# sonbui25/Multimodal-Aspect-Category-Sentiment-Analysis

Measured on AMD Instinct MI355X. Metric: train samples/sec (fwd+bwd+step) FCMF seq128x36ROI, higher is better.
Workload: dtype bf16; 1 GPU; FCMF-base fine-tune step, BASELINE configs[1]: batch 64 reviews x 6 aspects per GPU, seq 128, 7 images x (49 patches + 36 ROIs), precomputed ResNet-152 features, dropout 0.1, clip 1.0 + 4-group AdamW + linear schedule; global_batch=64, per_gpu_batch=64, seq_len=128, parallelism=dp1, sample_unit=1 review = 6 aspect forwards

## Files before the change

### multimodal-aspect-category-sentiment-analysis_amd/csrc/attn_mfma.hip

```cpp
#include "attn_tiles.h"
#include <cstdlib>


template <int NKT>
__device__ __forceinline__ void attn_mfma_fwd_tile(const AttnMfmaParams& P, int g, int h, int q0, int lane, const bf16x8 (&qf)[2][2],
                                                   const char* Ks, const char* Vs, const float* mask_lds = nullptr) {
  constexpr int NKF = 8 * NKT;
  const float* mrow = P.mask ? P.mask + (int64_t)g * P.Tk : nullptr;
  int nvalid = P.Tk;
  if (mask_lds || mrow) {
    int last = -1;
#pragma unroll
    for (int i = 0; i < 2 * NKT; ++i) {
      const int key = 64 * i + lane;
      const bool live = key < P.Tk && (mask_lds ? mask_lds[key] : mrow[key]) > -1e30f;
      const unsigned long long b = __ballot(live);
      if (b) last = 64 * i + 63 - __builtin_clzll(b);
    }
    nvalid = last >= 0 ? last + 1 : P.Tk;
  }
  f32x4 sc[NKF][2];
#pragma unroll
  for (int kf = 0; kf < NKF; ++kf)
#pragma unroll
    for (int f = 0; f < 2; ++f) sc[kf][f] = f32x4{0.f, 0.f, 0.f, 0.f};
#pragma unroll
  for (int s = 0; s < 2; ++s)
#pragma unroll
    for (int kf = 0; kf < NKF; ++kf) {
      if (16 * kf >= nvalid) continue;
      const bf16x8 ka = frag_row64(Ks, 16 * kf, s, lane);
#pragma unroll
      for (int f = 0; f < 2; ++f) sc[kf][f] = __builtin_amdgcn_mfma_f32_16x16x32_bf16(ka, qf[f][s], sc[kf][f], 0, 0, 0);
    }
  const float inv_keep = P.p > 0.f ? 1.0f / (1.0f - P.p) : 1.0f;
#pragma unroll
  for (int f = 0; f < 2; ++f) {
    const int q = q0 + 16 * f + (lane & 15);
    float m = -INFINITY;
#pragma unroll
    for (int kf = 0; kf < NKF; ++kf) {
      if (16 * kf >= nvalid) continue;
#pragma unroll
      for (int r = 0; r < 4; ++r) {
        const int key = 16 * kf + 4 * (lane >> 4) + r;
        float s = -INFINITY;
        if (key < P.Tk) s = sc[kf][f][r] * P.scale + (mask_lds ? mask_lds[key] : (mrow ? mrow[key] : 0.f));
        sc[kf][f][r] = s;
        m = fmaxf(m, s);
      }
    }
    m = fmaxf(m, __shfl_xor(m, 16, 64));
    m = fmaxf(m, __shfl_xor(m, 32, 64));
    float sum = 0.f;
#pragma unroll
    for (int kf = 0; kf < NKF; ++kf) {
      if (16 * kf >= nvalid) continue;
#pragma unroll
      for (int r = 0; r < 4; ++r) {
        const float e = __expf(sc[kf][f][r] - m);
        sc[kf][f][r] = e;
        sum += e;
      }
    }
    sum += __shfl_xor(sum, 16, 64);
    sum += __shfl_xor(sum, 32, 64);
    const float inv = 1.0f / sum;
    if (q < P.Tq && (lane >> 4) == 0 && P.lse) P.lse[((int64_t)g * P.heads + h) * P.Tq + q] = m + __logf(sum);
#pragma unroll
    for (int kf = 0; kf < NKF; ++kf) {
      if (16 * kf >= nvalid) continue;
      float dm[4] = {1.f, 1.f, 1.f, 1.f};
      if (P.p > 0.f)
        dropout_mult4(P.seed, ((uint64_t)g * P.heads + h) * P.Tq * P.Tk + (__umul24((unsigned)q, (unsigned)P.Tk) + (unsigned)(16 * kf + 4 * (lane >> 4))),
                      P.p, inv_keep, dm);
#pragma unroll
      for (int r = 0; r < 4; ++r) sc[kf][f][r] = sc[kf][f][r] * inv * dm[r];
    }
  }
  f32x4 oc[4][2];
#pragma unroll
  for (int df = 0; df < 4; ++df)
#pragma unroll
    for (int f = 0; f < 2; ++f) oc[df][f] = f32x4{0.f, 0.f, 0.f, 0.f};
#pragma unroll
  for (int s = 0; s < 4 * NKT; ++s) {
    if (32 * s >= nvalid) continue;
    bf16x8 pb[2];
#pragma unroll
    for (int f = 0; f < 2; ++f)
#pragma unroll
      for (int r = 0; r < 4; ++r) { pb[f][r] = (bf16_t)sc[2 * s][f][r]; pb[f][4 + r] = (bf16_t)sc[2 * s + 1][f][r]; }
#pragma unroll
    for (int df = 0; df < 4; ++df) {
      const bf16x8 va = frag_tr64p(Vs, 16 * df, s, lane);
#pragma unroll
      for (int f = 0; f < 2; ++f) oc[df][f] = __builtin_amdgcn_mfma_f32_16x16x32_bf16(va, pb[f], oc[df][f], 0, 0, 0);
    }
  }
#pragma unroll
  for (int f = 0; f < 2; ++f) {
    const int q = q0 + 16 * f + (lane & 15);
    if (q < P.Tq) {
      bf16_t* orow = P.out + ((int64_t)g * P.Tq + q) * P.ldo + h * AD + 4 * (lane >> 4);
#pragma unroll
      for (int df = 0; df < 4; ++df) store4(orow + 16 * df, oc[df][f]);
    }
  }
}

template <int NKT>
__device__ __forceinline__ void attn_mfma_fwd_body(const AttnMfmaParams& P) {
  extern __shared__ __attribute__((aligned(16))) char smem[];
  char* Ks = smem;
  char* Vs = smem + NKT * TILE_B;
  const int tid = threadIdx.x, lane = tid & 63, w = tid >> 6;
  const int g = blockIdx.x / P.heads, h = blockIdx.x % P.heads;
  const int q0 = blockIdx.y * AT + w * 32;
  const bf16_t* kbase_p = P.k + (int64_t)g * P.Tk * P.ldk + h * AD;
  const bf16_t* vbase_p = P.v + (int64_t)g * P.Tk * P.ldk + h * AD;
  const TileRegs kt = load_tile(kbase_p, P.ldk, P.Tk, tid);
  const TileRegs vt = load_tile(vbase_p, P.ldk, P.Tk, tid);
  bf16x8 qf[2][2];
  load_q_frags(P, g, h, q0, lane, qf);
  store_tile<false>(Ks, kt, tid);
  store_tile<true>(Vs, vt, tid);
  if constexpr (NKT == 2) {
    const TileRegs kt2 = load_tile(kbase_p + (int64_t)AT * P.ldk, P.ldk, P.Tk - AT, tid);
    const TileRegs vt2 = load_tile(vbase_p + (int64_t)AT * P.ldk, P.ldk, P.Tk - AT, tid);
    store_tile<false>(Ks + TILE_B, kt2, tid);
    store_tile<true>(Vs + TILE_B, vt2, tid);
  }
  __syncthreads();
  attn_mfma_fwd_tile<NKT>(P, g, h, q0, lane, qf, Ks, Vs);
}

__global__ __launch_bounds__(256, 2) void attn_mfma_fwd_persist_kernel(AttnMfmaParams P, int ntiles, int qtiles) {
  extern __shared__ __attribute__((aligned(16))) char smem[];
  const int tid = threadIdx.x, lane = tid & 63, w = tid >> 6;
  auto where = [&](int tile, int& g, int& h, int& q0) {
    const int gh = tile / qtiles;
    g = gh / P.heads; h = gh - g * P.heads; q0 = (tile - gh * qtiles) * AT + w * 32;
  };
  constexpr int BUF = 2 * TILE_B + 512;
  int tile = blockIdx.x;
  if (tile >= ntiles) return;
  int g, h, q0;
  where(tile, g, h, q0);
  bf16x8 qf[2][2];
  auto mask_of = [&](int gg) { return (P.mask && tid < P.Tk) ? P.mask[(int64_t)gg * P.Tk + tid] : 0.f; };
  {
    const TileRegs kt = load_tile(P.k + (int64_t)g * P.Tk * P.ldk + h * AD, P.ldk, P.Tk, tid);
    const TileRegs vt = load_tile(P.v + (int64_t)g * P.Tk * P.ldk + h * AD, P.ldk, P.Tk, tid);
    const float mv = mask_of(g);
    load_q_frags(P, g, h, q0, lane, qf);
    store_tile<false>(smem, kt, tid);
    store_tile<true>(smem + TILE_B, vt, tid);
    if (tid < AT) reinterpret_cast<float*>(smem + 2 * TILE_B)[tid] = mv;
  }
  __syncthreads();
  int cur = 0;
  for (;;) {
    const int nxt = tile + gridDim.x;
    const bool more = nxt < ntiles;
    int g2 = g, h2 = h, q2 = q0;
    TileRegs kt, vt;
    bf16x8 qn[2][2];
    float mv = 0.f;
    if (more) {
      where(nxt, g2, h2, q2);
      kt = load_tile(P.k + (int64_t)g2 * P.Tk * P.ldk + h2 * AD, P.ldk, P.Tk, tid);
      vt = load_tile(P.v + (int64_t)g2 * P.Tk * P.ldk + h2 * AD, P.ldk, P.Tk, tid);
      mv = mask_of(g2);
      load_q_frags(P, g2, h2, q2, lane, qn);
    }
    const char* buf = smem + cur * BUF;
    attn_mfma_fwd_tile<1>(P, g, h, q0, lane, qf, buf, buf + TILE_B, reinterpret_cast<const float*>(buf + 2 * TILE_B));
    if (!more) break;
    cur ^= 1;
    store_tile<false>(smem + cur * BUF, kt, tid);
    store_tile<true>(smem + cur * BUF + TILE_B, vt, tid);
    if (tid < AT) reinterpret_cast<float*>(smem + cur * BUF + 2 * TILE_B)[tid] = mv;
#pragma unroll
    for (int f = 0; f < 2; ++f)
#pragma unroll
      for (int s2 = 0; s2 < 2; ++s2) qf[f][s2] = qn[f][s2];
    g = g2; h = h2; q0 = q2; tile = nxt;
    __syncthreads();
  }
}

__global__ __launch_bounds__(256, 3) void attn_mfma_fwd_kernel(AttnMfmaParams P) { attn_mfma_fwd_body<1>(P); }
__global__ __launch_bounds__(256, 2) void attn_mfma_fwd256_kernel(AttnMfmaParams P) { attn_mfma_fwd_body<2>(P); }

template <int NQT, int NKT>
__device__ __forceinline__ void attn_mfma_bwd_body(const AttnMfmaParams& P) {
  extern __shared__ __attribute__((aligned(16))) char smem[];
  char* Qs = smem;
  char* dOs = Qs + NQT * TILE_B;
  char* Ks = dOs + NQT * TILE_B;
  char* Vs = Ks + NKT * TILE_B;
  char* PdT = Vs + NKT * TILE_B;
  char* dST = PdT + TILE_B / 2;
  const int tid = threadIdx.x, lane = tid & 63, w = tid >> 6;
  const int g = blockIdx.x / P.heads, h = blockIdx.x % P.heads;
  const int64_t qbase = (int64_t)g * P.Tq, kbase = (int64_t)g * P.Tk;
  float dl4[NQT][2][4], lse4[NQT][2][4];
  {
    TileRegs tq[NQT], td[NQT];
#pragma unroll
    for (int qt = 0; qt < NQT; ++qt) {
      tq[qt] = load_tile(P.q + (qbase + qt * AT) * P.ldq + h * AD, P.ldq, P.Tq - qt * AT, tid);
      td[qt] = load_tile(P.dout + (qbase + qt * AT) * P.ldo + h * AD, P.ldo, P.Tq - qt * AT, tid);
    }
    TileRegs tk = load_tile(P.k + kbase * P.ldk + h * AD, P.ldk, P.Tk, tid);
    TileRegs tv = load_tile(P.v + kbase * P.ldk + h * AD, P.ldk, P.Tk, tid);
#pragma unroll
    for (int qt = 0; qt < NQT; ++qt) {
      const int q = qt * AT + 32 * w + (lane >> 1), half = lane & 1;
      float sd = 0.f;
      if (q < P.Tq) {
        const bf16_t* a = P.dout + (qbase + q) * P.ldo + h * AD + 32 * half;
        const bf16_t* b = P.o + (qbase + q) * P.ldo + h * AD + 32 * half;
#pragma unroll
        for (int i = 0; i < 4; ++i) {
          const bf16x8 x = *reinterpret_cast<const bf16x8*>(a + 8 * i);
          const bf16x8 y = *reinterpret_cast<const bf16x8*>(b + 8 * i);
#pragma unroll
          for (int j = 0; j < 8; ++j) sd += (float)x[j] * (float)y[j];
        }
      }
      sd += __shfl_xor(sd, 1, 64);
#pragma unroll
      for (int f = 0; f < 2; ++f)
#pragma unroll
        for (int r = 0; r < 4; ++r) {
          const int ql = 16 * f + 4 * (lane >> 4) + r;
          dl4[qt][f][r] = __shfl(sd, 2 * ql, 64);
          const int q2 = qt * AT + 32 * w + ql;
          lse4[qt][f][r] = q2 < P.Tq ? P.lse[((int64_t)g * P.heads + h) * P.Tq + q2] : 0.f;
        }
    }
#pragma unroll
    for (int qt = 0; qt < NQT; ++qt) {
      store_tile<false>(Qs + qt * TILE_B, tq[qt], tid);
      store_tile<false>(dOs + qt * TILE_B, td[qt], tid);
    }
    store_tile<false>(Ks, tk, tid);
    store_tile<false>(Vs, tv, tid);
    if constexpr (NKT == 2) {
      tk = load_tile(P.k + (kbase + AT) * P.ldk + h * AD, P.ldk, P.Tk - AT, tid);
      tv = load_tile(P.v + (kbase + AT) * P.ldk + h * AD, P.ldk, P.Tk - AT, tid);
      store_tile<false>(Ks + TILE_B, tk, tid);
      store_tile<false>(Vs + TILE_B, tv, tid);
    }
  }
  __syncthreads();

  const float inv_keep = P.p > 0.f ? 1.0f / (1.0f - P.p) : 1.0f;
  const uint64_t drop_base = ((uint64_t)g * P.heads + h) * P.Tq * P.Tk;
  const float* mrow = P.mask ? P.mask + kbase : nullptr;
  float score_scale = P.scale;
  bf16x8 qa[NQT][2][2], da[NQT][2][2], oT[NQT][4], qT[NQT][4];
  f32x4 aQ[NQT][4][2];
#pragma unroll
  for (int qt = 0; qt < NQT; ++qt) {
#pragma unroll
    for (int f = 0; f < 2; ++f)
#pragma unroll
      for (int s = 0; s < 2; ++s) {
        qa[qt][f][s] = frag_row64(Qs + qt * TILE_B, 32 * w + 16 * f, s, lane);
        da[qt][f][s] = frag_row64(dOs + qt * TILE_B, 32 * w + 16 * f, s, lane);
// ... 114 lines not shown
      for (int s = 0; s < 4; ++s)
#pragma unroll
        for (int kf = 0; kf < 2; ++kf) {
          const bf16x8 pb = frag_row128(PdT, 16 * kf, s, lane);
          const bf16x8 sb = frag_row128(dST, 16 * kf, s, lane);
          aV[kf] = __builtin_amdgcn_mfma_f32_16x16x32_bf16(oT[qt][s], pb, aV[kf], 0, 0, 0);
          aK[kf] = __builtin_amdgcn_mfma_f32_16x16x32_bf16(qT[qt][s], sb, aK[kf], 0, 0, 0);
        }
      __syncthreads();
    }
    const int dcol = h * AD + 16 * w + 4 * (lane >> 4);
    cV += aV[0] + aV[1];
    cK += aK[0] + aK[1];
#pragma unroll
    for (int kf = 0; kf < 2; ++kf) {
      const int key = 32 * c + 16 * kf + (lane & 15);
      if (key < P.Tk) {
        store4(P.dv + (kbase + key) * P.ldk + dcol, aV[kf]);
        f32x4 t = aK[kf];
        t[0] *= P.scale; t[1] *= P.scale; t[2] *= P.scale; t[3] *= P.scale;
        store4(P.dk + (kbase + key) * P.ldk + dcol, t);
      }
    }
  }
  for (int c = nchunks; c < nchunks_all; ++c) {
    const int dcol = h * AD + 16 * w + 4 * (lane >> 4);
#pragma unroll
    for (int kf = 0; kf < 2; ++kf) {
      const int key = 32 * c + 16 * kf + (lane & 15);
      if (key < P.Tk) {
        store4(P.dv + (kbase + key) * P.ldk + dcol, f32x4{0.f, 0.f, 0.f, 0.f});
        store4(P.dk + (kbase + key) * P.ldk + dcol, f32x4{0.f, 0.f, 0.f, 0.f});
      }
    }
  }
#pragma unroll
  for (int qt = 0; qt < NQT; ++qt)
#pragma unroll
    for (int f = 0; f < 2; ++f) {
      const int x = qt * AT + 32 * w + 16 * f + (lane & 15);
      if (x < P.Tq) {
        const int dcol = h * AD + 4 * (lane >> 4);
#pragma unroll
        for (int df = 0; df < 4; ++df) {
          f32x4 t = aQ[qt][df][f];
          t[0] *= P.scale; t[1] *= P.scale; t[2] *= P.scale; t[3] *= P.scale;
          store4(P.dq + (qbase + x) * P.ldq + dcol + 16 * df, t);
        }
      }
    }
  if (P.colsum) {
    const int HD = P.heads * AD;
    float* row = P.colsum + (int64_t)g * 3 * HD + h * AD;
#pragma unroll
    for (int r = 0; r < 4; ++r) { cV[r] = row16_sum(cV[r]); cK[r] = row16_sum(cK[r]); }
    if ((lane & 15) == 0) {
      const int d0 = 16 * w + 4 * (lane >> 4);
#pragma unroll
      for (int r = 0; r < 4; ++r) { row[2 * HD + d0 + r] = cV[r]; row[HD + d0 + r] = cK[r] * P.scale; }
    }
    float* red = reinterpret_cast<float*>(PdT);
#pragma unroll
    for (int df = 0; df < 4; ++df) {
      f32x4 t = f32x4{0.f, 0.f, 0.f, 0.f};
#pragma unroll
      for (int qt = 0; qt < NQT; ++qt)
#pragma unroll
        for (int f = 0; f < 2; ++f) t += aQ[qt][df][f];
#pragma unroll
      for (int r = 0; r < 4; ++r) t[r] = row16_sum(t[r]);
      if ((lane & 15) == 0) {
#pragma unroll
        for (int r = 0; r < 4; ++r) red[w * 64 + 16 * df + 4 * (lane >> 4) + r] = t[r];
      }
    }
    __syncthreads();
    if (tid < 64) row[tid] = (red[tid] + red[64 + tid] + red[128 + tid] + red[192 + tid]) * P.scale;
  }
}

__global__ __launch_bounds__(256, 2) void attn_mfma_bwd_kernel(AttnMfmaParams P) { attn_mfma_bwd_body<1, 1>(P); }
__global__ __launch_bounds__(256, 1) void attn_mfma_bwd256_kernel(AttnMfmaParams P) { attn_mfma_bwd_body<2, 2>(P); }

static bool al16(const void* p) { return (reinterpret_cast<uintptr_t>(p) & 15) == 0; }

extern "C" int fcmf_attn_mfma_fwd(const void* q, const void* k, const void* v, const float* mask, void* out, float* lse,
                                  int G, int heads, int Tq, int Tk, int64_t ldq, int64_t ldk, int64_t ldo, float scale,
                                  float dropout_p, uint64_t seed, void* stream) {
  if (!q || !k || !v || !out || G <= 0 || heads <= 0 || Tq <= 0 || Tk <= 0) return FCMF_ERR_ARG;
  if (Tk > 2 * AT || ldq % 8 || ldk % 8 || ldo % 4 || !al16(q) || !al16(k) || !al16(v) || !al16(out)) return FCMF_ERR_UNSUPPORTED;
  AttnMfmaParams P{};
  P.q = (const bf16_t*)q; P.k = (const bf16_t*)k; P.v = (const bf16_t*)v; P.mask = mask; P.out = (bf16_t*)out; P.lse = lse;
  P.G = G; P.heads = heads; P.Tq = Tq; P.Tk = Tk; P.ldq = ldq; P.ldk = ldk; P.ldo = ldo;
  P.scale = scale; P.p = dropout_p; P.seed = seed;
  const dim3 grid(G * heads, (Tq + AT - 1) / AT);
  if (Tk > AT) {
    const int smem = 4 * TILE_B;
    static bool attr2 = false;
    return fcmf_launch_flagged(&attr2, attn_mfma_fwd256_kernel, grid, dim3(256), smem, reinterpret_cast<hipStream_t>(stream), P);
  }
  const int ntiles = (int)(grid.x * grid.y);
  static const bool no_persist = getenv("FCMF_ATTN_NO_PERSIST") != nullptr;
  if (ntiles >= 4 * 512 && !no_persist) {
    const int smem = 2 * (2 * TILE_B + 512);
    static bool attr3 = false;
    return fcmf_launch_flagged(&attr3, attn_mfma_fwd_persist_kernel, dim3(512), dim3(256), smem, reinterpret_cast<hipStream_t>(stream), P, ntiles, (int)grid.y);
  }
  const int smem = 2 * TILE_B;
  static bool attr = false;
  return fcmf_launch_flagged(&attr, attn_mfma_fwd_kernel, grid, dim3(256), smem, reinterpret_cast<hipStream_t>(stream), P);
}

extern "C" int fcmf_attn_mfma_bwd(const void* q, const void* k, const void* v, const float* mask, const void* out,
                                  const void* dout, const float* lse, void* dq, void* dk, void* dv, int G, int heads,
                                  int Tq, int Tk, int64_t ldq, int64_t ldk, int64_t ldo, float scale, float dropout_p,
                                  uint64_t seed, float* colsum, void* stream) {
  if (!q || !k || !v || !out || !dout || !lse || !dq || !dk || !dv || G <= 0 || heads <= 0 || Tq <= 0 || Tk <= 0) return FCMF_ERR_ARG;
  if (Tk > 2 * AT || Tq > 2 * AT || ldq % 8 || ldk % 8 || ldo % 8 || !al16(q) || !al16(k) || !al16(v) || !al16(out) || !al16(dout) ||
      !al16(dq) || !al16(dk) || !al16(dv))
    return FCMF_ERR_UNSUPPORTED;
  AttnMfmaParams P{};
  P.q = (const bf16_t*)q; P.k = (const bf16_t*)k; P.v = (const bf16_t*)v; P.mask = mask; P.o = (const bf16_t*)out;
  P.dout = (const bf16_t*)dout; P.lse = const_cast<float*>(lse); P.dq = (bf16_t*)dq; P.dk = (bf16_t*)dk; P.dv = (bf16_t*)dv;
  P.G = G; P.heads = heads; P.Tq = Tq; P.Tk = Tk; P.ldq = ldq; P.ldk = ldk; P.ldo = ldo;
  P.scale = scale; P.p = dropout_p; P.seed = seed; P.colsum = colsum;
  if (Tk > AT || Tq > AT) {
    const int smem = 9 * TILE_B;
    static bool attr2 = false;
    return fcmf_launch_flagged(&attr2, attn_mfma_bwd256_kernel, dim3(G * heads), dim3(256), smem, reinterpret_cast<hipStream_t>(stream), P);
  }
  const int smem = 5 * TILE_B;
  static bool attr = false;
  return fcmf_launch_flagged(&attr, attn_mfma_bwd_kernel, dim3(G * heads), dim3(256), smem, reinterpret_cast<hipStream_t>(stream), P);
}
```

### multimodal-aspect-category-sentiment-analysis_amd/csrc/attn_tiles.h

```cpp
#pragma once
#include "common.h"

constexpr int AD = 64;
constexpr int AT = 128;
constexpr int TILE_B = AT * AD * 2;

__device__ __forceinline__ int vkey(int r) { return ((r >> 1) & 1) | (((r >> 3) & 1) << 1); }
__device__ __forceinline__ int off64(int r, int c8) { return r * 128 + ((((c8 >> 1) ^ vkey(r))) << 5) + ((c8 & 1) << 4); }
__device__ __forceinline__ int key16(int r) { return ((r & 7) << 1) ^ (((r >> 3) & 1) * 9); }
__device__ __forceinline__ int off128(int r, int ch) { return r * 256 + ((ch ^ key16(r)) << 4); }
__device__ __forceinline__ int offp(int r, int ch) { return r * 256 + ((ch ^ (r & 15)) << 4); }

__device__ __forceinline__ int off64p(int r, int c8) { return r * 128 + ((((c8 >> 1) ^ ((r >> 1) & 3))) << 5) + ((c8 & 1) << 4); }

typedef bf16x4 __attribute__((address_space(3))) * lds_v4_t;

__device__ __forceinline__ void stage_tile(char* lds, const bf16_t* __restrict__ src, int64_t ld, int rows, int tid) {
#pragma unroll
  for (int i = 0; i < 4; ++i) {
    const int c = tid + 256 * i, r = c >> 3, c8 = c & 7;
    uint4 v = make_uint4(0, 0, 0, 0);
    if (r < rows) v = *reinterpret_cast<const uint4*>(src + (int64_t)r * ld + c8 * 8);
    *reinterpret_cast<uint4*>(lds + off64(r, c8)) = v;
  }
}
__device__ __forceinline__ void stage_tile_p(char* lds, const bf16_t* __restrict__ src, int64_t ld, int rows, int tid) {
#pragma unroll
  for (int i = 0; i < 4; ++i) {
    const int c = tid + 256 * i, r = c >> 3, c8 = c & 7;
    uint4 v = make_uint4(0, 0, 0, 0);
    if (r < rows) v = *reinterpret_cast<const uint4*>(src + (int64_t)r * ld + c8 * 8);
    *reinterpret_cast<uint4*>(lds + off64p(r, c8)) = v;
  }
}
__device__ __forceinline__ bf16x8 frag_tr64p(const char* lds, int c0, int s, int lane) {
  const int g4 = lane >> 4, i16 = lane & 15, q4 = i16 >> 2, p = i16 & 3;
  const int r = 32 * s + 4 * g4 + q4, c8 = (c0 >> 3) + (p >> 1);
  bf16x4 lo = __builtin_amdgcn_ds_read_tr16_b64_v4bf16((lds_v4_t)(lds + off64p(r, c8) + (p & 1) * 8));
  bf16x4 hi = __builtin_amdgcn_ds_read_tr16_b64_v4bf16((lds_v4_t)(lds + off64p(r + 16, c8) + (p & 1) * 8));
  bf16x8 o;
  o[0] = lo[0]; o[1] = lo[1]; o[2] = lo[2]; o[3] = lo[3]; o[4] = hi[0]; o[5] = hi[1]; o[6] = hi[2]; o[7] = hi[3];
  return o;
}
struct TileRegs { uint4 v[4]; };
__device__ __forceinline__ TileRegs load_tile(const bf16_t* __restrict__ src, int64_t ld, int rows, int tid) {
  TileRegs t;
#pragma unroll
  for (int i = 0; i < 4; ++i) {
    const int c = tid + 256 * i, r = c >> 3, c8 = c & 7;
    t.v[i] = make_uint4(0, 0, 0, 0);
    if (r < rows) t.v[i] = *reinterpret_cast<const uint4*>(src + (int64_t)r * ld + c8 * 8);
  }
  return t;
}
template <bool PERMUTED>
__device__ __forceinline__ void store_tile(char* lds, const TileRegs& t, int tid) {
#pragma unroll
  for (int i = 0; i < 4; ++i) {
    const int c = tid + 256 * i, r = c >> 3, c8 = c & 7;
    *reinterpret_cast<uint4*>(lds + (PERMUTED ? off64p(r, c8) : off64(r, c8))) = t.v[i];
  }
}
__device__ __forceinline__ bf16x8 frag_row64(const char* lds, int x0, int s, int lane) {
  return *reinterpret_cast<const bf16x8*>(lds + off64(x0 + (lane & 15), 4 * s + (lane >> 4)));
}
__device__ __forceinline__ bf16x8 frag_tr64(const char* lds, int c0, int s, int lane) {
  const int g4 = lane >> 4, i16 = lane & 15, q4 = i16 >> 2, p = i16 & 3;
  const int r = 32 * s + 8 * g4 + q4, c8 = (c0 >> 3) + (p >> 1);
  bf16x4 lo = __builtin_amdgcn_ds_read_tr16_b64_v4bf16((lds_v4_t)(lds + off64(r, c8) + (p & 1) * 8));
  bf16x4 hi = __builtin_amdgcn_ds_read_tr16_b64_v4bf16((lds_v4_t)(lds + off64(r + 4, c8) + (p & 1) * 8));
  bf16x8 o;
  o[0] = lo[0]; o[1] = lo[1]; o[2] = lo[2]; o[3] = lo[3]; o[4] = hi[0]; o[5] = hi[1]; o[6] = hi[2]; o[7] = hi[3];
  return o;
}
__device__ __forceinline__ bf16x8 frag_row128(const char* lds, int x0, int s, int lane) {
  return *reinterpret_cast<const bf16x8*>(lds + off128(x0 + (lane & 15), 4 * s + (lane >> 4)));
}
__device__ __forceinline__ bf16x8 frag_tr128(const char* lds, int c0, int s, int lane) {
  const int g4 = lane >> 4, i16 = lane & 15, q4 = i16 >> 2, p = i16 & 3;
  const int r = 32 * s + 8 * g4 + q4, ch = (c0 >> 3) + (p >> 1);
  bf16x4 lo = __builtin_amdgcn_ds_read_tr16_b64_v4bf16((lds_v4_t)(lds + off128(r, ch) + (p & 1) * 8));
  bf16x4 hi = __builtin_amdgcn_ds_read_tr16_b64_v4bf16((lds_v4_t)(lds + off128(r + 4, ch) + (p & 1) * 8));
  bf16x8 o;
  o[0] = lo[0]; o[1] = lo[1]; o[2] = lo[2]; o[3] = lo[3]; o[4] = hi[0]; o[5] = hi[1]; o[6] = hi[2]; o[7] = hi[3];
  return o;
}
__device__ __forceinline__ void store4(bf16_t* p, f32x4 v) {
  bf16x4 o;
  o[0] = (bf16_t)v[0]; o[1] = (bf16_t)v[1]; o[2] = (bf16_t)v[2]; o[3] = (bf16_t)v[3];
  *reinterpret_cast<bf16x4*>(p) = o;
}

__device__ __forceinline__ float row16_sum(float x) {
#define FCMF_ROR_ADD(n) x += __builtin_bit_cast(float, __builtin_amdgcn_update_dpp(0, __builtin_bit_cast(int, x), 0x120 + (n), 0xf, 0xf, true))
  FCMF_ROR_ADD(8); FCMF_ROR_ADD(4); FCMF_ROR_ADD(2); FCMF_ROR_ADD(1);
#undef FCMF_ROR_ADD
  return x;
}

struct AttnMfmaParams {
  const bf16_t *q, *k, *v, *o, *dout;
  const float* mask;
  bf16_t *out, *dq, *dk, *dv;
  float* lse;
  float* colsum;
  int G, heads, Tq, Tk;
  int64_t ldq, ldk, ldo;
  float scale, p;
  uint64_t seed;
};

__device__ __forceinline__ void load_q_frags(const AttnMfmaParams& P, int g, int h, int q0, int lane, bf16x8 (&qf)[2][2]) {
#pragma unroll
  for (int f = 0; f < 2; ++f)
#pragma unroll
    for (int s = 0; s < 2; ++s) {
      const int row = q0 + 16 * f + (lane & 15);
      uint4 v = make_uint4(0, 0, 0, 0);
      if (row < P.Tq) v = *reinterpret_cast<const uint4*>(P.q + ((int64_t)g * P.Tq + row) * P.ldq + h * AD + 32 * s + 8 * (lane >> 4));
      qf[f][s] = *reinterpret_cast<bf16x8*>(&v);
    }
}
```

### multimodal-aspect-category-sentiment-analysis_amd/fcmf_framework/ops.py

```python
import ctypes
import math
import os
import weakref

import torch

from . import _hip as H

_compute_dtype = torch.float32


def set_compute_dtype(dtype):
    global _compute_dtype
    if dtype not in (torch.float32, torch.bfloat16):
        raise ValueError("compute dtype must be torch.float32 or torch.bfloat16")
    _compute_dtype = dtype


def compute_dtype():
    return _compute_dtype


_fp8 = False

# ... 81 lines not shown
    def refresh_transposed(self):
        if not self.mapT:
            return
        self._prune_transposed()
        items = [(k, ent) for k, ent in self.mapT.items() if ent[3]]
        if not items:
            return
        sig = tuple((k[0], ent[0].data_ptr()) for k, ent in items)
        if self._mt_tables is None or self._mt_tables[0] != sig:
            dev = items[0][1][0].device
            desc = []
            for t, (k, ent) in enumerate(items):
                R, C = k[1]
                desc += [(t, r, c) for r in range((R + 63) // 64) for c in range((C + 63) // 64)]
            self._mt_tables = (sig,
                               torch.tensor([k[0] for k, _ in items], dtype=torch.int64, device=dev),
                               torch.tensor([ent[0].data_ptr() for _, ent in items], dtype=torch.int64, device=dev),
                               torch.tensor([list(k[1]) for k, _ in items], dtype=torch.int32, device=dev),
                               torch.tensor(desc, dtype=torch.int32, device=dev), len(desc))
        _, src, dst, dims, desc, n = self._mt_tables
        H.check(H.lib().fcmf_multi_cast_transpose(H.ptr(src), H.ptr(dst), H.ptr(dims), H.ptr(desc), n, H.stream()),
                "fcmf_multi_cast_transpose")
        for _, ent in items:
            ent[2] = False
            ent[1] = ent[4]()._version

    def head_nk(self, ws):
        key = tuple(w.data_ptr() for w in ws) + (tuple(ws[0].shape),)
        ent = self.mapH.get(key)
        if ent is None or any(r() is None for r in ent[2]):
            nh, E, d = ws[0].shape
            buf = torch.empty((len(ws) * nh * d, E), dtype=torch.bfloat16, device=ws[0].device)
            pieces = []
            for i, w in enumerate(ws):
                if w.dtype != torch.float32 or not w.is_contiguous() or tuple(w.shape) != (nh, E, d):
                    raise H.HipLibraryError("head_nk: dense float32 [n_head, E, d] parameters expected")
                for h in range(nh):
                    src, dst = w.detach()[h], buf[(i * nh + h) * d:(i * nh + h + 1) * d]
                    k2 = (src.data_ptr(), (E, d), key)
                    self.mapT[k2] = [dst, -1, True, True, weakref.ref(w), src.data_ptr() - w.data_ptr()]
                    pieces.append(k2)
            self._mt_tables = None
            ent = self.mapH[key] = (buf, pieces, [weakref.ref(w) for w in ws])
        buf, pieces, owners = ent
        for k2 in pieces:
            e = self.mapT.get(k2)
            if e is None or e[2] or e[1] != e[4]()._version:
                if e is None:
                    del self.mapH[key]
                    return self.head_nk(ws)
                self.refresh_transposed()
                break
        return buf

    def get_fp8(self, w, owner=None):
        key = (w.data_ptr(), tuple(w.shape))
        ent = self.mapQ.get(key)
        owner = w if owner is None else owner
        if ent is not None and ent[1] == w._version and not ent[2] and ent[3]() is owner:
            return ent[0]
        src = self.get(w) if w.is_contiguous() else w.detach().contiguous()
        q, sc = quant_fp8_rows(src, w.shape[0], w.shape[1], w.shape[1], out=None if ent is None else ent[0])
        self.mapQ[key] = [(q, sc), w._version, False, weakref.ref(owner)]
        return q, sc

    def get_fp8_t(self, w, owner=None):
        key = (w.data_ptr(), tuple(w.shape))
        ent = self.mapQT.get(key)
        owner = w if owner is None else owner
        if ent is not None and ent[1] == w._version and not ent[2] and ent[3]() is owner:
            return ent[0]
        wt = self.get_t(w, owner)
        q, sc = quant_fp8_rows(wt, wt.shape[0], wt.shape[1], wt.shape[1], out=None if ent is None else ent[0])
        self.mapQT[key] = [(q, sc), w._version, False, weakref.ref(owner)]
        return q, sc

    def padded(self, w):
        sh = self.get(w)
        return self.pad.get((w.data_ptr(), tuple(w.shape)), sh)

    def get(self, w):
        key = (w.data_ptr(), tuple(w.shape))
        ent = self.map.get(key)
        if ent is not None and ent[1] == w._version and not ent[2]:
            return ent[0]
        if ent is not None:
            sh = ent[0]
        elif w.dim() == 2 and w.shape[0] % VOCAB_PAD != 0:
            rows = (w.shape[0] + VOCAB_PAD - 1) // VOCAB_PAD * VOCAB_PAD
            full = torch.zeros((rows, w.shape[1]), dtype=torch.bfloat16, device=w.device)
            sh = full[:w.shape[0]]
            self.pad[key] = full
        else:
            sh = torch.empty(w.shape, dtype=torch.bfloat16, device=w.device)
        src = w.detach()
        if not src.is_contiguous():
            src = src.contiguous()
        H.check(H.lib().fcmf_cast(H.ptr(src), H.ptr(sh), src.numel(), H.F32, H.BF16, H.stream()), "fcmf_cast")
        self.map[key] = [sh, w._version, False]
        return sh

    def derived(self, w, tag, build):
        key = (w.data_ptr(), tuple(w.shape), tag)
        ent = self.mapD.get(key)
        if ent is not None and ent[1] == w._version and not ent[2]:
            return ent[0]
        t = build(w.detach())
        self.mapD[key] = [t, w._version, False]
        return t

    def peek(self, w):
        ent = self.map.get((w.data_ptr(), tuple(w.shape)))
        return None if ent is None else ent[0]

    def mark_fresh(self, w):
        ent = self.map.get((w.data_ptr(), tuple(w.shape)))
        if ent is not None:
            ent[1] = w._version
            ent[2] = False

    def mark_all_stale(self):
        for ent in self.map.values():
            ent[2] = True
        for ent in self.mapT.values():
            ent[2] = True
        for ent in self.mapD.values():
            ent[2] = True
        for m in (self.mapQ, self.mapQT):
            for k in [k for k, ent in m.items() if ent[3]() is None]:
                del m[k]
            for ent in m.values():
                ent[2] = True

    def clear(self):
        self.map.clear()
        self.pad.clear()
        self.mapT.clear()
        self.mapD.clear()
        self.mapQ.clear()
        self.mapQT.clear()
        self.mapH.clear()
        self._mt_tables = None


shadows = _Shadows()

_grad_arena = None


def set_grad_arena(arena):
    global _grad_arena
    _grad_arena = arena
    if arena is not None and deferred_dw.reset not in arena.on_zero:
        arena.on_zero.append(deferred_dw.reset)


def grad_arena():
    return _grad_arena


def grad_dest(param, shape, *, rows=None, in_place=True, temp=True, device=None):
    a = _grad_arena
    if a is not None and param is not None:
        if isinstance(param, (list, tuple)):
            ok = all(q.dtype == torch.float32 and q.is_contiguous() for q in param) and sum(q.numel() for q in param) == math.prod(shape)
        else:
            ok = param.dtype == torch.float32 and param.is_contiguous() and param.numel() == math.prod(shape)
        got = a.claim(param, rows) if ok else None
        if got is not None and (got[1] or in_place):
            buf, first = got
            if rows is None:
                buf = buf.view(shape)
                return buf, (buf if first else None)
            return buf, (a.grad_alias(param, shape) if first else None)
    if not temp:
        return None, None
    if device is None:
        device = (param[0] if isinstance(param, (list, tuple)) else param).device
    if rows is None:
        buf = torch.zeros(shape, dtype=torch.float32, device=device)
        return buf, buf
    buf = torch.zeros((rows,) + tuple(shape[1:]), dtype=torch.float32, device=device)
    return buf, buf[:shape[0]]


def as_compute(w, dtype):
    if dtype == torch.float32:
        return w.detach()
    return shadows.get(w)


# ... 1223 lines not shown
```

Before: 1734 samples/s.

## Use 8-wave attention fwd persistent and bwd kernels by default

Adds 512-thread (8-wave) variants of the persistent forward attention kernel and the backward attention kernel. In forward each wave handles fewer query rows, and in backward the waves split dK and dV computation. The goal is more waves per CU to hide latency and spread the per-head work. An env var keeps the old 4-wave kernels available. The weight-cache lookups also gain weakref ownership checks, which fix stale-cache reuse but add a little host overhead.

```diff
diff --git a/multimodal-aspect-category-sentiment-analysis_amd/csrc/attn_mfma.hip b/multimodal-aspect-category-sentiment-analysis_amd/csrc/attn_mfma.hip
--- a/multimodal-aspect-category-sentiment-analysis_amd/csrc/attn_mfma.hip
+++ b/multimodal-aspect-category-sentiment-analysis_amd/csrc/attn_mfma.hip
@@ -2,8 +2,8 @@
 #include <cstdlib>
 
 
-template <int NKT>
-__device__ __forceinline__ void attn_mfma_fwd_tile(const AttnMfmaParams& P, int g, int h, int q0, int lane, const bf16x8 (&qf)[2][2],
+template <int NKT, int NF>
+__device__ __forceinline__ void attn_mfma_fwd_tile(const AttnMfmaParams& P, int g, int h, int q0, int lane, const bf16x8 (&qf)[NF][2],
                                                    const char* Ks, const char* Vs, const float* mask_lds = nullptr) {
   constexpr int NKF = 8 * NKT;
   const float* mrow = P.mask ? P.mask + (int64_t)g * P.Tk : nullptr;
@@ -19,11 +19,11 @@
     }
     nvalid = last >= 0 ? last + 1 : P.Tk;
   }
-  f32x4 sc[NKF][2];
+  f32x4 sc[NKF][NF];
 #pragma unroll
   for (int kf = 0; kf < NKF; ++kf)
 #pragma unroll
-    for (int f = 0; f < 2; ++f) sc[kf][f] = f32x4{0.f, 0.f, 0.f, 0.f};
+    for (int f = 0; f < NF; ++f) sc[kf][f] = f32x4{0.f, 0.f, 0.f, 0.f};
 #pragma unroll
   for (int s = 0; s < 2; ++s)
 #pragma unroll
@@ -31,11 +31,11 @@
       if (16 * kf >= nvalid) continue;
       const bf16x8 ka = frag_row64(Ks, 16 * kf, s, lane);
 #pragma unroll
-      for (int f = 0; f < 2; ++f) sc[kf][f] = __builtin_amdgcn_mfma_f32_16x16x32_bf16(ka, qf[f][s], sc[kf][f], 0, 0, 0);
+      for (int f = 0; f < NF; ++f) sc[kf][f] = __builtin_amdgcn_mfma_f32_16x16x32_bf16(ka, qf[f][s], sc[kf][f], 0, 0, 0);
     }
   const float inv_keep = P.p > 0.f ? 1.0f / (1.0f - P.p) : 1.0f;
 #pragma unroll
-  for (int f = 0; f < 2; ++f) {
+  for (int f = 0; f < NF; ++f) {
     const int q = q0 + 16 * f + (lane & 15);
     float m = -INFINITY;
 #pragma unroll
@@ -78,28 +78,28 @@
       for (int r = 0; r < 4; ++r) sc[kf][f][r] = sc[kf][f][r] * inv * dm[r];
     }
   }
-  f32x4 oc[4][2];
+  f32x4 oc[4][NF];
 #pragma unroll
   for (int df = 0; df < 4; ++df)
 #pragma unroll
-    for (int f = 0; f < 2; ++f) oc[df][f] = f32x4{0.f, 0.f, 0.f, 0.f};
+    for (int f = 0; f < NF; ++f) oc[df][f] = f32x4{0.f, 0.f, 0.f, 0.f};
 #pragma unroll
   for (int s = 0; s < 4 * NKT; ++s) {
     if (32 * s >= nvalid) continue;
-    bf16x8 pb[2];
-#pragma unroll
-    for (int f = 0; f < 2; ++f)
+    bf16x8 pb[NF];
+#pragma unroll
+    for (int f = 0; f < NF; ++f)
 #pragma unroll
       for (int r = 0; r < 4; ++r) { pb[f][r] = (bf16_t)sc[2 * s][f][r]; pb[f][4 + r] = (bf16_t)sc[2 * s + 1][f][r]; }
 #pragma unroll
     for (int df = 0; df < 4; ++df) {
       const bf16x8 va = frag_tr64p(Vs, 16 * df, s, lane);
 #pragma unroll
-      for (int f = 0; f < 2; ++f) oc[df][f] = __builtin_amdgcn_mfma_f32_16x16x32_bf16(va, pb[f], oc[df][f], 0, 0, 0);
-    }
-  }
-#pragma unroll
-  for (int f = 0; f < 2; ++f) {
+      for (int f = 0; f < NF; ++f) oc[df][f] = __builtin_amdgcn_mfma_f32_16x16x32_bf16(va, pb[f], oc[df][f], 0, 0, 0);
+    }
+  }
+#pragma unroll
+  for (int f = 0; f < NF; ++f) {
     const int q = q0 + 16 * f + (lane & 15);
     if (q < P.Tq) {
       bf16_t* orow = P.out + ((int64_t)g * P.Tq + q) * P.ldo + h * AD + 4 * (lane >> 4);
@@ -132,26 +132,30 @@
     store_tile<true>(Vs + TILE_B, vt2, tid);
   }
   __syncthreads();
-  attn_mfma_fwd_tile<NKT>(P, g, h, q0, lane, qf, Ks, Vs);
-}
-
-__global__ __launch_bounds__(256, 2) void attn_mfma_fwd_persist_kernel(AttnMfmaParams P, int ntiles, int qtiles) {
+  attn_mfma_fwd_tile<NKT, 2>(P, g, h, q0, lane, qf, Ks, Vs);
+}
+
+template <int NW>
+__device__ __forceinline__ void attn_mfma_fwd_persist_body(const AttnMfmaParams& P, int ntiles, int qtiles) {
+  constexpr int NT = 64 * NW, NF = 8 / NW;
   extern __shared__ __attribute__((aligned(16))) char smem[];
-  const int tid = threadIdx.x, lane = tid & 63, w = tid >> 6;
+  const int tid = threadIdx.x, lane = tid & 63;
+  int w = tid >> 6;
+  if constexpr (NW == 8) w = __builtin_amdgcn_readfirstlane(w);
   auto where = [&](int tile, int& g, int& h, int& q0) {
     const int gh = tile / qtiles;
-    g = gh / P.heads; h = gh - g * P.heads; q0 = (tile - gh * qtiles) * AT + w * 32;
+    g = gh / P.heads; h = gh - g * P.heads; q0 = (tile - gh * qtiles) * AT + w * (16 * NF);
   };
   constexpr int BUF = 2 * TILE_B + 512;
   int tile = blockIdx.x;
   if (tile >= ntiles) return;
   int g, h, q0;
   where(tile, g, h, q0);
-  bf16x8 qf[2][2];
+  bf16x8 qf[NF][2];
   auto mask_of = [&](int gg) { return (P.mask && tid < P.Tk) ? P.mask[(int64_t)gg * P.Tk + tid] : 0.f; };
   {
-    const TileRegs kt = load_tile(P.k + (int64_t)g * P.Tk * P.ldk + h * AD, P.ldk, P.Tk, tid);
-    const TileRegs vt = load_tile(P.v + (int64_t)g * P.Tk * P.ldk + h * AD, P.ldk, P.Tk, tid);
+    const TileRegsT<NT> kt = load_tile<NT>(P.k + (int64_t)g * P.Tk * P.ldk + h * AD, P.ldk, P.Tk, tid);
+    const TileRegsT<NT> vt = load_tile<NT>(P.v + (int64_t)g * P.Tk * P.ldk + h * AD, P.ldk, P.Tk, tid);
     const float mv = mask_of(g);
     load_q_frags(P, g, h, q0, lane, qf);
     store_tile<false>(smem, kt, tid);
@@ -164,30 +168,39 @@
     const int nxt = tile + gridDim.x;
     const bool more = nxt < ntiles;
     int g2 = g, h2 = h, q2 = q0;
-    TileRegs kt, vt;
-    bf16x8 qn[2][2];
+    TileRegsT<NT> kt, vt;
+    bf16x8 qn[NF][2];
     float mv = 0.f;
     if (more) {
       where(nxt, g2, h2, q2);
-      kt = load_tile(P.k + (int64_t)g2 * P.Tk * P.ldk + h2 * AD, P.ldk, P.Tk, tid);
-      vt = load_tile(P.v + (int64_t)g2 * P.Tk * P.ldk + h2 * AD, P.ldk, P.Tk, tid);
+      kt = load_tile<NT>(P.k + (int64_t)g2 * P.Tk * P.ldk + h2 * AD, P.ldk, P.Tk, tid);
+      vt = load_tile<NT>(P.v + (int64_t)g2 * P.Tk * P.ldk + h2 * AD, P.ldk, P.Tk, tid);
       mv = mask_of(g2);
       load_q_frags(P, g2, h2, q2, lane, qn);
     }
     const char* buf = smem + cur * BUF;
-    attn_mfma_fwd_tile<1>(P, g, h, q0, lane, qf, buf, buf + TILE_B, reinterpret_cast<const float*>(buf + 2 * TILE_B));
+    int tl = lane;
+    if constexpr (NW == 8) asm volatile("" : "+v"(tl));
+    attn_mfma_fwd_tile<1, NF>(P, g, h, q0, tl, qf, buf, buf + TILE_B, reinterpret_cast<const float*>(buf + 2 * TILE_B));
     if (!more) break;
     cur ^= 1;
     store_tile<false>(smem + cur * BUF, kt, tid);
     store_tile<true>(smem + cur * BUF + TILE_B, vt, tid);
     if (tid < AT) reinterpret_cast<float*>(smem + cur * BUF + 2 * TILE_B)[tid] = mv;
 #pragma unroll
-    for (int f = 0; f < 2; ++f)
+    for (int f = 0; f < NF; ++f)
 #pragma unroll
       for (int s2 = 0; s2 < 2; ++s2) qf[f][s2] = qn[f][s2];
     g = g2; h = h2; q0 = q2; tile = nxt;
     __syncthreads();
   }
+}
+
+__global__ __launch_bounds__(256, 2) void attn_mfma_fwd_persist_kernel(AttnMfmaParams P, int ntiles, int qtiles) {
+  attn_mfma_fwd_persist_body<4>(P, ntiles, qtiles);
+}
+__global__ __launch_bounds__(512, 4) void attn_mfma_fwd_persist8_kernel(AttnMfmaParams P, int ntiles, int qtiles) {
+  attn_mfma_fwd_persist_body<8>(P, ntiles, qtiles);
 }
 
 __global__ __launch_bounds__(256, 3) void attn_mfma_fwd_kernel(AttnMfmaParams P) { attn_mfma_fwd_body<1>(P); }
@@ -468,7 +481,244 @@
 __global__ __launch_bounds__(256, 2) void attn_mfma_bwd_kernel(AttnMfmaParams P) { attn_mfma_bwd_body<1, 1>(P); }
 __global__ __launch_bounds__(256, 1) void attn_mfma_bwd256_kernel(AttnMfmaParams P) { attn_mfma_bwd_body<2, 2>(P); }
 
+__device__ __forceinline__ void attn_mfma_bwd8_body(const AttnMfmaParams& P) {
+  constexpr int NT = 512;
+  extern __shared__ __attribute__((aligned(16))) char smem[];
+  char* Qs = smem;
+  char* dOs = Qs + TILE_B;
+  char* Ks = dOs + TILE_B;
+  char* Vs = Ks + TILE_B;
+  char* PdT = Vs + TILE_B;
+  char* dST = PdT + TILE_B / 2;
+  const int tid = threadIdx.x, lane = tid & 63;
+  const int w = __builtin_amdgcn_readfirstlane(tid >> 6);
+  const int g = blockIdx.x / P.heads, h = blockIdx.x % P.heads;
+  const int64_t qbase = (int64_t)g * P.Tq, kbase = (int64_t)g * P.Tk;
+  float dl4[4], lse4[4];
+  {
+    const TileRegsT<NT> tq = load_tile<NT>(P.q + qbase * P.ldq + h * AD, P.ldq, P.Tq, tid);
+    const TileRegsT<NT> td = load_tile<NT>(P.dout + qbase * P.ldo + h * AD, P.ldo, P.Tq, tid);
+    const TileRegsT<NT> tk = load_tile<NT>(P.k + kbase * P.ldk + h * AD, P.ldk, P.Tk, tid);
+    const TileRegsT<NT> tv = load_tile<NT>(P.v + kbase * P.ldk + h * AD, P.ldk, P.Tk, tid);
+    const int q = 16 * w + (lane >> 1), half = lane & 1;
+    float sd = 0.f;
+    if (lane < 32 && q < P.Tq) {
+      const bf16_t* a = P.dout + (qbase + q) * P.ldo + h * AD + 32 * half;
+      const bf16_t* b = P.o + (qbase + q) * P.ldo + h * AD + 32 * half;
+#pragma unroll
+      for (int i = 0; i < 4; ++i) {
+        const bf16x8 x = *reinterpret_cast<const bf16x8*>(a + 8 * i);
+        const bf16x8 y = *reinterpret_cast<const bf16x8*>(b + 8 * i);
+#pragma unroll
+        for (int j = 0; j < 8; ++j) sd += (float)x[j] * (float)y[j];
+      }
+    }
+    sd += __shfl_xor(sd, 1, 64);
+#pragma unroll
+    for (int r = 0; r < 4; ++r) {
+      const int ql = 4 * (lane >> 4) + r;
+      dl4[r] = __shfl(sd, 2 * ql, 64);
+      const int q2 = 16 * w + ql;
+      lse4[r] = q2 < P.Tq ? P.lse[((int64_t)g * P.heads + h) * P.Tq + q2] : 0.f;
+    }
+    store_tile<false>(Qs, tq, tid);
+    store_tile<false>(dOs, td, tid);
+    store_tile<false>(Ks, tk, tid);
+    store_tile<false>(Vs, tv, tid);
+  }
+  __syncthreads();
+
+  const float inv_keep = P.p > 0.f ? 1.0f / (1.0f - P.p) : 1.0f;
+  const uint64_t drop_base = ((uint64_t)g * P.heads + h) * P.Tq * P.Tk;
+  const float* mrow = P.mask ? P.mask + kbase : nullptr;
+  float score_scale = P.scale;
+  const bool isV = w < 4;
+  const int wc = w & 3;
+  const char* Timg = isV ? dOs : Qs;
+  const char* Cimg = isV ? PdT : dST;
+  bf16_t* const kvout = isV ? P.dv : P.dk;
+  const float kvscale = isV ? 1.0f : P.scale;
+  bf16x8 qa[2], da[2], xT[4];
+  f32x4 aQ[4];
+#pragma unroll
+  for (int s = 0; s < 2; ++s) {
+    qa[s] = frag_row64(Qs, 16 * w, s, lane);
+    da[s] = frag_row64(dOs, 16 * w, s, lane);
+  }
+#pragma unroll
+  for (int s = 0; s < 4; ++s) xT[s] = frag_tr64(Timg, 16 * wc, s, lane);
+#pragma unroll
+  for (int df = 0; df < 4; ++df) aQ[df] = f32x4{0.f, 0.f, 0.f, 0.f};
+
+  const int nchunks_all = (P.Tk + 31) >> 5;
+  int nvalid = P.Tk;
+  if (mrow) {
+    int last = -1;
+#pragma unroll
+    for (int i = 0; i < 2; ++i) {
+      const int key = 64 * i + lane;
+      const bool live = key < P.Tk && mrow[key] > -1e30f;
+      const unsigned long long b = __ballot(live);
+      if (b) last = 64 * i + 63 - __builtin_clzll(b);
+    }
+    nvalid = last >= 0 ? last + 1 : P.Tk;
+    if (last < 0) {
+      mrow = nullptr;
+      score_scale = 0.f;
+      const float ltk = __logf((float)P.Tk);
+#pragma unroll
+      for (int r = 0; r < 4; ++r) lse4[r] = ltk;
+    }
+  }
+  const int nchunks = (nvalid + 31) >> 5;
+  const uint64_t pair_base = drop_base >> 1;
+  const uint32_t pb_lo = (uint32_t)pair_base, pb_hi = (uint32_t)(pair_base >> 32);
+  const bool share_hash = P.p > 0.f && (P.Tk & 1) == 0 && pb_lo <= 0xFFFF0000u;
+  const uint32_t hash_k0 = (uint32_t)P.seed ^ ((pb_hi << 7) | (pb_hi >> 25)), hash_s1 = (uint32_t)(P.seed >> 32);
+  const uint32_t drop_thr = dropout_threshold(P.p);
+  const int odd = lane & 1;
+  f32x4 cX = f32x4{0.f, 0.f, 0.f, 0.f};
+  for (int c = 0; c < nchunks; ++c) {
+    f32x4 aX[2];
+#pragma unroll
+    for (int kf = 0; kf < 2; ++kf) aX[kf] = f32x4{0.f, 0.f, 0.f, 0.f};
+    f32x4 sS[2], sP[2];
+#pragma unroll
+    for (int k4 = 0; k4 < 2; ++k4) { sS[k4] = f32x4{0.f, 0.f, 0.f, 0.f}; sP[k4] = f32x4{0.f, 0.f, 0.f, 0.f}; }
+#pragma unroll
+    for (int s = 0; s < 2; ++s)
+#pragma unroll
+      for (int k4 = 0; k4 < 2; ++k4) {
+        const bf16x8 kb = frag_row64(Ks, 32 * c + 16 * k4, s, lane);
+        const bf16x8 vb = frag_row64(Vs, 32 * c + 16 * k4, s, lane);
+        sS[k4] = __builtin_amdgcn_mfma_f32_16x16x32_bf16(qa[s], kb, sS[k4], 0, 0, 0);
+        sP[k4] = __builtin_amdgcn_mfma_f32_16x16x32_bf16(da[s], vb, sP[k4], 0, 0, 0);
+      }
+#pragma unroll
+    for (int k4 = 0; k4 < 2; ++k4) {
+      const int kl = 16 * k4 + (lane & 15), key = 32 * c + kl;
+      const float mk = (mrow && key < P.Tk) ? mrow[key] : 0.f;
+      f32x4 pdv, dsv;
+      float mult4[4] = {1.0f, 1.0f, 1.0f, 1.0f};
+      if (share_hash) {
+        const unsigned q0 = 16 * w + 4 * (lane >> 4);
+        const uint32_t o0 = pb_lo + __umul24(q0 + 2 * odd, (unsigned)P.Tk >> 1) + ((unsigned)key >> 1);
+        const uint32_t hA = fcmf_hash32_rounds(o0 ^ hash_k0, hash_s1);
+        const uint32_t hB = fcmf_hash32_rounds((o0 + ((unsigned)P.Tk >> 1)) ^ hash_k0, hash_s1);
+        const uint32_t nA = (uint32_t)__builtin_amdgcn_update_dpp(0, (int)hA, 0xB1, 0xf, 0xf, true);
+        const uint32_t nB = (uint32_t)__builtin_amdgcn_update_dpp(0, (int)hB, 0xB1, 0xf, 0xf, true);
+        const uint32_t hr[4] = {odd ? nA : hA, odd ? nB : hB, odd ? hA : nA, odd ? hB : nB};
+#pragma unroll
+        for (int r = 0; r < 4; ++r) mult4[r] = ((hr[r] >> (16 * odd)) & 0xFFFFu) >= drop_thr ? inv_keep : 0.f;
+      }
+#pragma unroll
+      for (int r = 0; r < 4; ++r) {
+        const int q = 16 * w + 4 * (lane >> 4) + r;
+        float pr = 0.f, mult = mult4[r];
+        if (key < P.Tk && q < P.Tq) pr = __expf(sS[k4][r] * score_scale + mk - lse4[r]);
+        if (P.p > 0.f && !share_hash) mult = dropout_mult(P.seed, drop_base + (__umul24((unsigned)q, (unsigned)P.Tk) + (unsigned)key), P.p, inv_keep);
+        pdv[r] = pr * mult;
+        dsv[r] = pr * (sP[k4][r] * mult - dl4[r]);
+      }
+      const int ch = 2 * w + (lane >> 5);
+      const int o = off128(kl, ch) + ((lane >> 4) & 1) * 8;
+      store4(reinterpret_cast<bf16_t*>(PdT + o), pdv);
+      store4(reinterpret_cast<bf16_t*>(dST + o), dsv);
+    }
+    __syncthreads();
+    {
+      const bf16x8 tb = frag_tr128(dST, 16 * w, 0, lane);
+#pragma unroll
+      for (int df = 0; df < 4; ++df) {
+        const bf16x8 ka2 = frag_tr64(Ks, 16 * df, c, lane);
+        aQ[df] = __builtin_amdgcn_mfma_f32_16x16x32_bf16(ka2, tb, aQ[df], 0, 0, 0);
+      }
+    }
+#pragma unroll
+    for (int s = 0; s < 4; ++s)
+#pragma unroll
+      for (int kf = 0; kf < 2; ++kf) {
+        const bf16x8 xb = frag_row128(Cimg, 16 * kf, s, lane);
+        aX[kf] = __builtin_amdgcn_mfma_f32_16x16x32_bf16(xT[s], xb, aX[kf], 0, 0, 0);
+      }
+    __syncthreads();
+    cX += aX[0] + aX[1];
+    int sl = lane;
+    asm volatile("" : "+v"(sl));
+#pragma unroll
+    for (int kf = 0; kf < 2; ++kf) {
+      const int key = 32 * c + 16 * kf + (sl & 15);
+      if (key < P.Tk) {
+        f32x4 t = aX[kf];
+        t[0] *= kvscale; t[1] *= kvscale; t[2] *= kvscale; t[3] *= kvscale;
+        store4(kvout + (kbase + key) * P.ldk + h * AD + 16 * wc + 4 * (sl >> 4), t);
+      }
+    }
+  }
+  int el = lane;
+  asm volatile("" : "+v"(el));
+  for (int c = nchunks; c < nchunks_all; ++c) {
+#pragma unroll
+    for (int kf = 0; kf < 2; ++kf) {
+      const int key = 32 * c + 16 * kf + (el & 15);
+      if (key < P.Tk) store4(kvout + (kbase + key) * P.ldk + h * AD + 16 * wc + 4 * (el >> 4), f32x4{0.f, 0.f, 0.f, 0.f});
+    }
+  }
+  {
+    const int x = 16 * w + (el & 15);
+    if (x < P.Tq) {
+      const int dq0 = h * AD + 4 * (el >> 4);
+#pragma unroll
+      for (int df = 0; df < 4; ++df) {
+        f32x4 t = aQ[df];
+        t[0] *= P.scale; t[1] *= P.scale; t[2] *= P.scale; t[3] *= P.scale;
+        store4(P.dq + (qbase + x) * P.ldq + dq0 + 16 * df, t);
+      }
+    }
+  }
+  if (P.colsum) {
+    const int HD = P.heads * AD;
+    float* row = P.colsum + (int64_t)g * 3 * HD + h * AD;
+#pragma unroll
+    for (int r = 0; r < 4; ++r) cX[r] = row16_sum(cX[r]);
+    if ((el & 15) == 0) {
+      const int d0 = (isV ? 2 * HD : HD) + 16 * wc + 4 * (el >> 4);
+#pragma unroll
+      for (int r = 0; r < 4; ++r) row[d0 + r] = cX[r] * kvscale;
+    }
+    f32x4* xch = reinterpret_cast<f32x4*>(PdT);
+    float* red = reinterpret_cast<float*>(Qs);
+    if (w & 1) {
+#pragma unroll
+      for (int df = 0; df < 4; ++df) xch[((w >> 1) * 4 + df) * 64 + el] = aQ[df];
+    }
+    __syncthreads();
+    if (!(w & 1)) {
+#pragma unroll
+      for (int df = 0; df < 4; ++df) {
+        f32x4 t = f32x4{0.f, 0.f, 0.f, 0.f};
+        t += aQ[df];
+        t += xch[((w >> 1) * 4 + df) * 64 + el];
+#pragma unroll
+        for (int r = 0; r < 4; ++r) t[r] = row16_sum(t[r]);
+        if ((el & 15) == 0) {
+#pragma unroll
+          for (int r = 0; r < 4; ++r) red[(w >> 1) * 64 + 16 * df + 4 * (el >> 4) + r] = t[r];
+        }
+      }
+    }
+    __syncthreads();
+    if (tid < 64) row[tid] = (red[tid] + red[64 + tid] + red[128 + tid] + red[192 + tid]) * P.scale;
+  }
+}
+
+__global__ __launch_bounds__(512, 4) void attn_mfma_bwd8_kernel(AttnMfmaParams P) { attn_mfma_bwd8_body(P); }
+
 static bool al16(const void* p) { return (reinterpret_cast<uintptr_t>(p) & 15) == 0; }
+static bool attn_four_waves() {
+  const char* e = getenv("FCMF_ATTN_WAVES");
+  return e && atoi(e) == 4;
+}
 
 extern "C" int fcmf_attn_mfma_fwd(const void* q, const void* k, const void* v, const float* mask, void* out, float* lse,
                                   int G, int heads, int Tq, int Tk, int64_t ldq, int64_t ldk, int64_t ldo, float scale,
@@ -489,8 +739,10 @@
   static const bool no_persist = getenv("FCMF_ATTN_NO_PERSIST") != nullptr;
   if (ntiles >= 4 * 512 && !no_persist) {
     const int smem = 2 * (2 * TILE_B + 512);
-    static bool attr3 = false;
-    return fcmf_launch_flagged(&attr3, attn_mfma_fwd_persist_kernel, dim3(512), dim3(256), smem, reinterpret_cast<hipStream_t>(stream), P, ntiles, (int)grid.y);
+    static bool attr3 = false, attr4 = false;
+    if (attn_four_waves())
+      return fcmf_launch_flagged(&attr3, attn_mfma_fwd_persist_kernel, dim3(512), dim3(256), smem, reinterpret_cast<hipStream_t>(stream), P, ntiles, (int)grid.y);
+    return fcmf_launch_flagged(&attr4, attn_mfma_fwd_persist8_kernel, dim3(512), dim3(512), smem, reinterpret_cast<hipStream_t>(stream), P, ntiles, (int)grid.y);
   }
   const int smem = 2 * TILE_B;
   static bool attr = false;
@@ -516,6 +768,8 @@
     return fcmf_launch_flagged(&attr2, attn_mfma_bwd256_kernel, dim3(G * heads), dim3(256), smem, reinterpret_cast<hipStream_t>(stream), P);
   }
   const int smem = 5 * TILE_B;
-  static bool attr = false;
-  return fcmf_launch_flagged(&attr, attn_mfma_bwd_kernel, dim3(G * heads), dim3(256), smem, reinterpret_cast<hipStream_t>(stream), P);
-}
+  static bool attr = false, attr8 = false;
+  if (attn_four_waves())
+    return fcmf_launch_flagged(&attr, attn_mfma_bwd_kernel, dim3(G * heads), dim3(256), smem, reinterpret_cast<hipStream_t>(stream), P);
+  return fcmf_launch_flagged(&attr8, attn_mfma_bwd8_kernel, dim3(G * heads), dim3(512), smem, reinterpret_cast<hipStream_t>(stream), P);
+}
diff --git a/multimodal-aspect-category-sentiment-analysis_amd/csrc/attn_tiles.h b/multimodal-aspect-category-sentiment-analysis_amd/csrc/attn_tiles.h
--- a/multimodal-aspect-category-sentiment-analysis_amd/csrc/attn_tiles.h
+++ b/multimodal-aspect-category-sentiment-analysis_amd/csrc/attn_tiles.h
@@ -42,22 +42,24 @@
   o[0] = lo[0]; o[1] = lo[1]; o[2] = lo[2]; o[3] = lo[3]; o[4] = hi[0]; o[5] = hi[1]; o[6] = hi[2]; o[7] = hi[3];
   return o;
 }
-struct TileRegs { uint4 v[4]; };
-__device__ __forceinline__ TileRegs load_tile(const bf16_t* __restrict__ src, int64_t ld, int rows, int tid) {
-  TileRegs t;
+template <int NT = 256> struct TileRegsT { uint4 v[1024 / NT]; };
+typedef TileRegsT<256> TileRegs;
+template <int NT = 256>
+__device__ __forceinline__ TileRegsT<NT> load_tile(const bf16_t* __restrict__ src, int64_t ld, int rows, int tid) {
+  TileRegsT<NT> t;
 #pragma unroll
-  for (int i = 0; i < 4; ++i) {
-    const int c = tid + 256 * i, r = c >> 3, c8 = c & 7;
+  for (int i = 0; i < 1024 / NT; ++i) {
+    const int c = tid + NT * i, r = c >> 3, c8 = c & 7;
     t.v[i] = make_uint4(0, 0, 0, 0);
     if (r < rows) t.v[i] = *reinterpret_cast<const uint4*>(src + (int64_t)r * ld + c8 * 8);
   }
   return t;
 }
-template <bool PERMUTED>
-__device__ __forceinline__ void store_tile(char* lds, const TileRegs& t, int tid) {
+template <bool PERMUTED, int NT = 256>
+__device__ __forceinline__ void store_tile(char* lds, const TileRegsT<NT>& t, int tid) {
 #pragma unroll
-  for (int i = 0; i < 4; ++i) {
-    const int c = tid + 256 * i, r = c >> 3, c8 = c & 7;
+  for (int i = 0; i < 1024 / NT; ++i) {
+    const int c = tid + NT * i, r = c >> 3, c8 = c & 7;
     *reinterpret_cast<uint4*>(lds + (PERMUTED ? off64p(r, c8) : off64(r, c8))) = t.v[i];
   }
 }
@@ -110,9 +112,10 @@
   uint64_t seed;
 };
 
-__device__ __forceinline__ void load_q_frags(const AttnMfmaParams& P, int g, int h, int q0, int lane, bf16x8 (&qf)[2][2]) {
+template <int NF>
+__device__ __forceinline__ void load_q_frags(const AttnMfmaParams& P, int g, int h, int q0, int lane, bf16x8 (&qf)[NF][2]) {
 #pragma unroll
-  for (int f = 0; f < 2; ++f)
+  for (int f = 0; f < NF; ++f)
 #pragma unroll
     for (int s = 0; s < 2; ++s) {
       const int row = q0 + 16 * f + (lane & 15);
diff --git a/multimodal-aspect-category-sentiment-analysis_amd/fcmf_framework/ops.py b/multimodal-aspect-category-sentiment-analysis_amd/fcmf_framework/ops.py
--- a/multimodal-aspect-category-sentiment-analysis_amd/fcmf_framework/ops.py
+++ b/multimodal-aspect-category-sentiment-analysis_amd/fcmf_framework/ops.py
@@ -187,7 +187,9 @@
     def get(self, w):
         key = (w.data_ptr(), tuple(w.shape))
         ent = self.map.get(key)
-        if ent is not None and ent[1] == w._version and not ent[2]:
+        par = isinstance(w, torch.nn.Parameter)
+        if ent is not None and ent[1] == w._version and not ent[2] and (
+                ent[3] is None or (ent[3]() is w if par else ent[3]() is not None)):
             return ent[0]
         if ent is not None:
             sh = ent[0]
@@ -202,16 +204,16 @@
         if not src.is_contiguous():
             src = src.contiguous()
         H.check(H.lib().fcmf_cast(H.ptr(src), H.ptr(sh), src.numel(), H.F32, H.BF16, H.stream()), "fcmf_cast")
-        self.map[key] = [sh, w._version, False]
+        self.map[key] = [sh, w._version, False, weakref.ref(w) if par else None]
         return sh
 
     def derived(self, w, tag, build):
         key = (w.data_ptr(), tuple(w.shape), tag)
         ent = self.mapD.get(key)
-        if ent is not None and ent[1] == w._version and not ent[2]:
+        if ent is not None and ent[1] == w._version and not ent[2] and ent[3]() is w:
             return ent[0]
         t = build(w.detach())
-        self.mapD[key] = [t, w._version, False]
+        self.mapD[key] = [t, w._version, False, weakref.ref(w)]
         return t
 
     def peek(self, w):
```

Result: no change. 1750 samples/s, median of 6 (+0.9%).
